# acerbilab/pyvbmc

Measured on AMD Instinct MI355X. Metric: ELBO+entropy evals/sec at D=10, K=50, N=400, Ns=1e6 (1e6-sample-equivalent evals/s), higher is better.
Workload: dtype f64; 1 GPU; BASELINE config 3 per GPU: D=10 K=50 N=400 S=1, Ns=1000000 MC samples per GPU (job Ns=1000000), value+grad _neg_elcbo with soft bounds, eps=philox; parallelism=single GPU

## Files before the change

### pyvbmc_amd/build.py

```python
import os
import subprocess
import sys
from pathlib import Path

HERE = Path(__file__).resolve().parent
CSRC = HERE / "csrc"
LIB = HERE / "libvbmc_hip.so"
SOURCES = [
    "ctx.hip",
    "entropy.hip",
    "entropy_small.hip",
    "prep.hip",
    "api_entropy.hip",
    "mixture.hip",
    "gp.hip",
    "api_gp.hip",
    "gp_post.hip",
    "api_gp_post.hip",
    "gp_lml.hip",
    "api_gp_lml.hip",
    "lockstep.hip",
    "gp_hyp.hip",
    "api_gp_hyp.hip",
    "gp_opt.hip",
    "api_gp_opt.hip",
    "gp_fit.hip",
    "api_gp_fit.hip",
    "api_elbo.hip",
    "api_batch.hip",
    "adam.hip",
    "adam_fused.hip",
    "api_acq.hip",
    "api_acq_is.hip",
    "acq_is_prep.hip",
    "acq_is_mcmc.hip",
    "search.hip",
    "api_search.hip",
    "sieve.hip",
    "api_sieve.hip",
    "elcbo_full.hip",
    "api_elcbo_full.hip",
    "cmaes.hip",
    "api_cmaes.hip",
    "sample.hip",
    "transform.hip",
    "kde.hip",
    "mode.hip",
    "warp.hip",
    "api_warp.hip",
    "comm.hip",
    "host_randn.hip",
    "device_randn.hip",
]
PROBE_SRC = CSRC / "devprobe.hip"
PROBE_LIB = HERE / "libvbmc_devprobe.so"
HIPCC = os.environ.get("HIPCC", "/opt/rocm/bin/hipcc")
FLAGS = [
    "--offload-arch=gfx950",
    "-O3",
    "-std=c++17",
    "-fPIC",
    "-ffp-contract=off",
    "-Wall",
    "-Wno-unused-function",
    "-Werror=pass-failed",
]


WS_DPS = [2, 4, 6, 8, 10, 12, 16, 20, 24, 32]
MFMA_DPS = [12, 16, 20, 24, 32]
WS_EXTRA = os.environ.get("VBMC_WS_EXTRA_FLAGS", "").split()
ALL_EXTRA = os.environ.get("VBMC_EXTRA_FLAGS", "").split()


def _sources():
    return [CSRC / s for s in SOURCES if (CSRC / s).exists()]


SOURCE_FLAGS = {}


def _jobs(bdir):
    jobs = [(src, bdir / (src.stem + ".o"), list(ALL_EXTRA) + SOURCE_FLAGS.get(src.name, [])) for src in _sources()]
    for dp in WS_DPS:
        jobs.append((CSRC / "entropy_ws.hip", bdir / f"entropy_ws_dp{dp}.o", [f"-DVBMC_DP={dp}"] + WS_EXTRA))
    for dp in MFMA_DPS:
        jobs.append((CSRC / "entropy_mfma.hip", bdir / f"entropy_mfma_dp{dp}.o", [f"-DVBMC_MFMA_DP={dp}"] + ALL_EXTRA))
    return jobs


def _headers():
    return list(CSRC.glob("*.h")) + [HERE.parent / "include" / "vbmc_hip.h"]


def _stale(lib, deps):
    return not lib.exists() or any(p.stat().st_mtime > lib.stat().st_mtime for p in deps)


def _lib_stale():
    return _stale(LIB, _sources() + [CSRC / "entropy_ws.hip", CSRC / "entropy_mfma.hip"] + _headers())


def _probe_stale():
    return _stale(PROBE_LIB, [PROBE_SRC] + _headers())


def needs_build():
    return _lib_stale() or _probe_stale()


def build_probe(verbose=True):
    cmd = [HIPCC, *FLAGS, *ALL_EXTRA, "-shared", str(PROBE_SRC), "-o", str(PROBE_LIB), "-Wl,-rpath,/opt/rocm/lib"]
    if verbose:
        print(" ".join(cmd), flush=True)
    subprocess.check_call(cmd)
    return PROBE_LIB


def build(force=False, verbose=True):
    if force or _probe_stale():
        build_probe(verbose)
    if not force and not _lib_stale():
        return LIB
    objs = []
    procs = []
    bdir = CSRC / "_obj"
    bdir.mkdir(exist_ok=True)
    import concurrent.futures as cf

    def run(job):
        src, obj, extra = job
        cmd = [HIPCC, *FLAGS, *extra, "-c", str(src), "-o", str(obj)]
        if verbose:
            print(" ".join(cmd), flush=True)
        p = subprocess.run(cmd, stdout=subprocess.PIPE, stderr=subprocess.STDOUT)
        return obj, p

    jobs = _jobs(bdir)
    with cf.ThreadPoolExecutor(max_workers=max(2, (os.cpu_count() or 4))) as ex:
        results = list(ex.map(run, jobs))
    for (src, obj, _), (_, p) in zip(jobs, results):
        objs.append(obj)
        procs.append((obj, p))
    failed = False
    for src, p in procs:
        out = p.stdout
        if p.returncode != 0:
            failed = True
            sys.stderr.write(f"--- {src.name} failed ---\n{out.decode()}\n")
        elif verbose and out.strip():
            sys.stderr.write(out.decode())
    if failed:
        raise RuntimeError("hipcc failed")
    cmd = [HIPCC, "--offload-arch=gfx950", "-shared", "-fPIC", *map(str, objs), "-o", str(LIB),
           "-ldl", "-Wl,-rpath,/opt/rocm/lib"]
    if verbose:
        print(" ".join(cmd), flush=True)
    subprocess.check_call(cmd)
    return LIB


if __name__ == "__main__":
    build(force="--force" in sys.argv)
    print(LIB)
    print(PROBE_LIB)
```

### pyvbmc_amd/variational_optimization.py

```python
import ctypes as C
import math
import os

import numpy as np

from . import _lib
from ._duck import ctx_of, optimize_mask, upload_vp
from .entropy import DEFAULT_RNG, _even_ns, entlb_vbmc, entmc_vbmc, philox_seed, upload_reference_eps
from .gp import upload_gp


def _soft_bound_loss(x, slb, sub, tol_con=1e-3, compute_grad=False):
    x = np.asarray(x, dtype=np.float64)
    ell = (sub - slb) * tol_con
    below = x < slb
    above = x > sub
    y = 0.0
    dy = np.zeros(x.shape)
    if np.any(below):
        y += 0.5 * np.sum(((slb[below] - x[below]) / ell[below]) ** 2)
        dy[below] = (x[below] - slb[below]) / ell[below] ** 2
    if np.any(above):
        y += 0.5 * np.sum(((x[above] - sub[above]) / ell[above]) ** 2)
        dy[above] = (x[above] - sub[above]) / ell[above] ** 2
    return (y, dy) if compute_grad else y


def _vp_bound_loss(vp, theta, theta_bnd, tol_con=1e-3, compute_grad=True):
    D, K = vp.D, vp.K
    pos = 0
    if vp.optimize_mu:
        mu = theta[: D * K]
        pos = D * K
    else:
        mu = vp.mu.ravel(order="F")
    if vp.optimize_sigma:
        ln_sigma = theta[pos : pos + K]
        pos += K
    else:
        ln_sigma = np.log(vp.sigma.ravel())
    ln_lambd = theta[pos : pos + D] if vp.optimize_lambd else np.log(vp.lambd.ravel())
    ln_scale = np.reshape(ln_lambd, (-1, 1)) + np.reshape(ln_sigma, (1, -1))
    parts = []
    if vp.optimize_mu:
        parts.append(np.ravel(mu))
    if vp.optimize_sigma or vp.optimize_lambd:
        parts.append(ln_scale.ravel(order="F"))
    if vp.optimize_weights:
        parts.append(np.ravel(theta[-K:]))
    ext = np.concatenate(parts)
    lb, ub = theta_bnd["lb"].ravel(), theta_bnd["ub"].ravel()
    if not compute_grad:
        return _soft_bound_loss(ext, lb, ub, tol_con)
    L, dL = _soft_bound_loss(ext, lb, ub, tol_con, compute_grad=True)
    out = []
    pos = 0
    if vp.optimize_mu:
        out.append(dL[: D * K])
        pos = D * K
    if vp.optimize_sigma or vp.optimize_lambd:
        block = np.reshape(dL[pos : pos + D * K], (D, K))
        if vp.optimize_sigma:
            out.append(block.sum(axis=0))
        if vp.optimize_lambd:
            out.append(block.sum(axis=1))
    if vp.optimize_weights:
        out.append(dL[-K:])
    return L, np.concatenate(out)


def _gp_log_joint(vp, gp, grad_flags, avg_flag=True, jacobian_flag=True, compute_var=False,
                  separate_K=False, *, ctx=None):
    if np.isscalar(grad_flags):
        grad_flags = (bool(grad_flags),) * 4
    bits = _lib.flags_to_bits(grad_flags)
    ctx = ctx_of(vp, ctx)
    upload_vp(vp, ctx)
    upload_gp(gp, ctx)
    D, K, S = vp.D, vp.K, len(gp.posteriors)
    jac = bool(jacobian_flag)
    n_dG = (D * K * bool(bits & 1) + jac * (K * bool(bits & 2) + D * bool(bits & 4) + K * bool(bits & 8)))
    averaged = S > 1 and avg_flag
    G = np.empty(S)
    dG = np.empty((n_dG, S)) if bits else None
    varG = np.empty(S) if compute_var else None
    var_ss = C.c_double(0.0)
    I_sk = np.empty((S, K)) if separate_K else None
    J_sjk = np.empty((S, K, K)) if (separate_K and compute_var) else None
    ctx.check(
        ctx._lib.vbmc_gp_log_joint(
            ctx._h, bits, int(bool(avg_flag)), int(jac), int(compute_var), _lib.ptr(G),
            _lib.ptr(dG), _lib.ptr(varG), C.byref(var_ss), _lib.ptr(I_sk), _lib.ptr(J_sjk),
        )
    )
    if averaged:
        G_out = G[0]
        dG_out = dG.ravel()[:n_dG].copy() if bits else None
        varG_out = varG[0] if compute_var else None
    else:
        G_out = G[0] if S == 1 else G
        dG_out = (dG[:, 0].copy() if S == 1 else dG) if bits else None
        varG_out = varG if compute_var else None
    vss = var_ss.value if (averaged and compute_var) else 0
    if separate_K:
        return G_out, dG_out, varG_out, None, vss, I_sk, J_sjk
    return G_out, dG_out, varG_out, None, vss


def _neg_elcbo(theta, gp, vp, beta=0.0, Ns=0, compute_grad=True, compute_var=None, theta_bnd=None,
               _entropy_alpha=0.0, separate_K=False, *, rng=None, seed=None, eps_half=None, ctx=None,
               rows=None):
    fs = _fast_last[0]
    if (fs is not None and fs.vp is vp and fs.gp is gp and fs.bnd is theta_bnd and Ns == fs.Ns and beta == 0.0
            and compute_grad is fs.cg and not compute_var and not separate_K and ctx is fs.ctx_arg and rng == fs.rng
            and eps_half is None and rows is None and type(theta) is np.ndarray and theta.size == fs.n_theta):
        rc = fs.call(theta, seed)
        if rc is not None:
            return rc
    _fast_last[0] = None
    if not math.isfinite(beta):
        beta = 0
    if compute_var is None:
        compute_var = beta != 0
    if compute_grad and beta != 0 and compute_var != 2:
        raise NotImplementedError(
            "Computation of the gradient of ELBO with full variance not supported"
        )
    if separate_K and compute_grad:
        raise ValueError(
            "Computing the gradient of variational parameters and "
            "requesting per-component results at the same time."
        )
    ctx_arg = ctx
    ctx = ctx_of(vp, ctx)
    K, D = vp.K, vp.D

    if separate_K or compute_var or beta != 0:
        if rows is not None:
            raise ValueError("rows= is only supported by the fused evaluation")
        return _neg_elcbo_composed(theta, gp, vp, beta, Ns, compute_grad, compute_var, theta_bnd,
                                   separate_K, rng, seed, eps_half, ctx)

    mask = optimize_mask(vp)
    if mask != 15 or getattr(ctx, "D", None) != D or getattr(ctx, "K", None) != K:
        upload_vp(vp, ctx)
    upload_gp(gp, ctx, lazy=True)
    n_theta = theta.size if type(theta) is np.ndarray else np.size(theta)
    fc = _fused_call(ctx, D, K, n_theta, theta_bnd)
    fc.th[:] = theta
    opts = fc.opts
    ns = _even_ns(Ns) if Ns > 0 else 0
    mode = 0
    if ns > 0:
        mode = DEFAULT_RNG if rng is None else rng
        if rows is not None and (eps_half is not None or mode != "philox"):
            raise ValueError("rows= needs rng='philox' (uploaded draws follow the context's own share)")
        if eps_half is not None or mode == "numpy":
            upload_reference_eps(ctx, K, D, ns, eps_half)
            mode, seed = _lib.EPS_RESIDENT, 0
        elif mode == "philox":
            if seed is None:
                seed = philox_seed(ctx)
            mode = _lib.EPS_PHILOX
        else:
            raise ValueError(f"unknown rng {mode!r}")
    shape = (ns, 1 if compute_grad else 0, mask, mode, rows)
    if shape != fc.shape:
        opts.ns_per_comp, opts.compute_grad, opts.optimize_mask = ns, shape[1], mask
        opts.row_begin, opts.row_count = (0, -1) if rows is None else (int(rows[0]), int(rows[1]))
        opts.eps_mode = mode
        fc.shape = shape
    if ns > 0:
        opts.seed = seed
    fc.side = (vp, theta, mask, K)
    try:
        rc = fc.fn(*fc.args)
        if rc != 0:
            if rc == _lib.W_GP_CHANGED:
                upload_gp(gp, ctx)
                rc = fc.fn(*fc.args)
            if rc != 0:
                ctx.check(rc)
        if fc.side is not None:
            fc.apply_side_effects()
    finally:
        fc.side = None
    if rows is None and eps_half is None and (ns == 0 or mode == _lib.EPS_PHILOX) and type(compute_grad) is bool:
        _fast_last[0] = _FastElbo(ctx_arg, ctx, fc, vp, gp, theta_bnd, Ns, compute_grad, rng, mask, D, K, n_theta, mode)
    return fc.F.value, (fc.dF.copy() if compute_grad else None), fc.G.value, fc.H.value, 0


def _neg_elcbo_batch(thetas, gp, vp, theta_bnd=None, *, ctx=None, return_parts=False):
    ctx = ctx_of(vp, ctx)
    thetas = np.ascontiguousarray(np.atleast_2d(thetas), dtype=np.float64)
    B, n_theta = thetas.shape
    upload_vp(vp, ctx)
    upload_gp(gp, ctx)
    opts = _lib.ElboOpts()
    opts.ns_per_comp, opts.compute_grad, opts.optimize_mask = 0, 0, optimize_mask(vp)
    keep = []
    if theta_bnd is not None:
        lb, ub = _lib.f64(theta_bnd["lb"].ravel()), _lib.f64(theta_bnd["ub"].ravel())
        keep += [lb, ub]
        opts.bnd_lb, opts.bnd_ub, opts.n_bnd = _lib.ptr(lb), _lib.ptr(ub), lb.size
        opts.tol_con = float(theta_bnd["tol_con"])
        opts.weight_threshold = float(theta_bnd.get("weight_threshold", 0.0))
        opts.weight_penalty = float(theta_bnd.get("weight_penalty", 0.0))
    F, G, H = np.empty(B), np.empty(B), np.empty(B)
    ctx.check(
        ctx._lib.vbmc_neg_elcbo_batch(
            ctx._h, _lib.ptr(thetas), B, n_theta, C.byref(opts), _lib.ptr(F), _lib.ptr(G), _lib.ptr(H)
        )
    )
    return (F, G, H) if return_parts else F


_RELEASE_CB = os.environ.get("VBMC_RELEASE_CB", "1") != "0"
_FAST_PATH = os.environ.get("VBMC_FAST_PATH", "1") != "0"
_fast_last = [None]


def clear_fast_path():
    _fast_last[0] = None


class _FastElbo:

    __slots__ = ("ctx_arg", "ctx", "fc", "vp", "gp", "bnd", "Ns", "cg", "rng", "mask", "D", "K", "n_theta", "philox",
                 "lb", "ub", "tol", "wthr", "wpen", "fused_last")

    def __init__(self, ctx_arg, ctx, fc, vp, gp, bnd, Ns, cg, rng, mask, D, K, n_theta, mode):
        self.ctx_arg, self.ctx, self.fc, self.vp, self.gp, self.bnd = ctx_arg, ctx, fc, vp, gp, bnd
        self.Ns, self.cg, self.rng, self.mask, self.D, self.K, self.n_theta = Ns, cg, rng, mask, D, K, n_theta
        self.philox = Ns > 0 and mode == _lib.EPS_PHILOX
        self.fused_last = ctx.__dict__.get("_fused_last")
        if bnd is not None:
            self.lb, self.ub = bnd["lb"], bnd["ub"]
            self.tol, self.wthr, self.wpen = bnd["tol_con"], bnd.get("weight_threshold", 0.0), bnd.get("weight_penalty", 0.0)
            if not fc.direct:
                self.vp = None

    def call(self, theta, seed):
        if not _FAST_PATH:
            return None
        vp, ctx, fc, bnd = self.vp, self.ctx, self.fc, self.bnd
        if (((1 if vp.optimize_mu else 0) | (2 if vp.optimize_sigma else 0) | (4 if vp.optimize_lambd else 0)
             | (8 if vp.optimize_weights else 0)) != self.mask or vp.D != self.D or vp.K != self.K
                or ctx.__dict__.get("_fused_last") is not self.fused_last or getattr(ctx, "D", None) != self.D
                or getattr(ctx, "K", None) != self.K or ctx_of(vp, self.ctx_arg) is not ctx):
            return None
        if self.mask != 15:
            return None
        if bnd is not None and (bnd["lb"] is not self.lb or bnd["ub"] is not self.ub or bnd["tol_con"] != self.tol
                                or bnd.get("weight_threshold", 0.0) != self.wthr or bnd.get("weight_penalty", 0.0) != self.wpen):
            return None
        gp = self.gp
        ps, X = gp.posteriors, gp.X
        quick = [id(ps), id(X), X.shape[0]]
        for p in ps:
            quick += (id(p), id(p.alpha), id(p.hyp))
        if quick != ctx.__dict__.get("_gp_quick"):
            return None
        fc.th[:] = theta
        if self.philox:
            fc.opts.seed = philox_seed(ctx) if seed is None else seed
        fc.side = (vp, theta, self.mask, self.K)
        try:
            rc = fc.fn(*fc.args)
            if rc != 0:
                if rc == _lib.W_GP_CHANGED:
                    upload_gp(gp, ctx)
                    rc = fc.fn(*fc.args)
                if rc != 0:
                    ctx.check(rc)
            if fc.side is not None:
                fc.apply_side_effects()
        finally:
            fc.side = None
        return fc.F.value, (fc.dF.copy() if self.cg else None), fc.G.value, fc.H.value, 0


class _FusedCall:

    def __init__(self, ctx, D, K, n_theta):
        self.th = np.empty(n_theta)
        self.dF = np.empty(n_theta)
        self.mu = np.empty((K, D))
        self.sg, self.lm, self.w, self.eta = np.empty(K), np.empty(D), np.empty(K), np.empty(K)
        self.mu_T, self.sg_row, self.lm_col = self.mu.T, self.sg.reshape(1, -1), self.lm.reshape(-1, 1)
        self.w_row, self.eta_row = self.w.reshape(1, -1), self.eta.reshape(1, -1)
        self.F, self.G, self.H = C.c_double(), C.c_double(), C.c_double()
        o = self.opts = _lib.ElboOpts()
        o.row_begin, o.row_count, o.seed = 0, -1, 0
        self.shape = None
        self.lb_src = self.ub_src = self.lb = self.ub = None
        self.fn = ctx._lib.vbmc_neg_elcbo_call
        self.side = None
        self._cb = C.CFUNCTYPE(None, C.c_void_p)(self._released)
        dp = C.POINTER(C.c_double)
        self.block = _lib.ElboCall(
            _lib.ptr(self.th), n_theta, C.pointer(o), C.cast(C.pointer(self.F), dp), _lib.ptr(self.dF),
            C.cast(C.pointer(self.G), dp), C.cast(C.pointer(self.H), dp), _lib.ptr(self.mu), _lib.ptr(self.sg),
            _lib.ptr(self.lm), _lib.ptr(self.w), _lib.ptr(self.eta),
        )
        self.args = (ctx._h, C.byref(self.block))
        if os.environ.get("VBMC_ELBO_CALL_BLOCK", "1") == "0":
            self.fn = ctx._lib.vbmc_neg_elcbo
            self.args = (
                ctx._h, _lib.ptr(self.th), n_theta, C.byref(o), C.byref(self.F), _lib.ptr(self.dF),
                C.byref(self.G), C.byref(self.H), _lib.ptr(self.mu), _lib.ptr(self.sg), _lib.ptr(self.lm),
                _lib.ptr(self.w), _lib.ptr(self.eta),
            )

    def apply_side_effects(self):
        vp, theta, mask, K = self.side
        vp.mu, vp.sigma, vp.lambd, vp.w = self.mu_T.copy(), self.sg_row.copy(), self.lm_col.copy(), self.w_row.copy()
        if mask & 8:
            vp.eta = self.eta_row.copy()
            if type(theta) is np.ndarray and theta.dtype == self.th.dtype:
                theta[-K:] = self.th[-K:]
        if hasattr(vp, "_mode"):
            vp._mode = None
        self.side = None

    def _released(self, _user):
        if self.side is not None:
            try:
                self.apply_side_effects()
            except Exception:
                pass

    def bind_bounds(self, theta_bnd):
        o = self.opts
        if theta_bnd is None:
            if self.lb is not None:
                o.bnd_lb, o.bnd_ub, o.n_bnd = None, None, 0
                self.lb_src = self.ub_src = self.lb = self.ub = None
            return
        lb, ub = theta_bnd["lb"], theta_bnd["ub"]
        if lb is not self.lb_src or ub is not self.ub_src:
            self.lb, self.ub = _lib.f64(np.ravel(lb)), _lib.f64(np.ravel(ub))
            self.direct = np.shares_memory(self.lb, lb) and np.shares_memory(self.ub, ub)
            self.lb_src, self.ub_src = (lb, ub) if self.direct else (None, None)
            o.bnd_lb, o.bnd_ub, o.n_bnd = _lib.ptr(self.lb), _lib.ptr(self.ub), self.lb.size
        o.tol_con = float(theta_bnd["tol_con"])
        o.weight_threshold = float(theta_bnd.get("weight_threshold", 0.0))
        o.weight_penalty = float(theta_bnd.get("weight_penalty", 0.0))


def _fused_call(ctx, D, K, n_theta, theta_bnd):
    last = ctx.__dict__.get("_fused_last")
    if last is not None and last[0] == D and last[1] == K and last[2] == n_theta:
        fc = last[3]
        fc.bind_bounds(theta_bnd)
        return fc
    cache = ctx.__dict__.setdefault("_fused_cache", {})
    key = (D, K, n_theta)
    fc = cache.get(key)
    if fc is None:
        if len(cache) > 16:
            cache.clear()
        fc = cache[key] = _FusedCall(ctx, D, K, n_theta)
    ctx.__dict__["_fused_last"] = (D, K, n_theta, fc)
    ctx.check(ctx._lib.vbmc_set_release_callback(ctx._h, C.cast(fc._cb, C.c_void_p) if _RELEASE_CB else None, None))
    fc.bind_bounds(theta_bnd)
    return fc


def _neg_elcbo_composed(theta, gp, vp, beta, Ns, compute_grad, compute_var, theta_bnd, separate_K,
                        rng, seed, eps_half, ctx):
    K = vp.K
    vp.set_parameters(theta)
    if vp.optimize_weights:
        tail = theta[-K:]
        tail -= np.amax(tail)
        vp.eta = np.reshape(tail, (1, -1))
    if compute_grad:
        grad_flags = (vp.optimize_mu, vp.optimize_sigma, vp.optimize_lambd, vp.optimize_weights)
    else:
        grad_flags = (False,) * 4
    I_sk = J_sjk = None
    dG = dvarG = None
    if separate_K:
        if compute_var:
            G, _, varG, _, varG_ss, I_sk, J_sjk = _gp_log_joint(vp, gp, grad_flags, 1, 1, compute_var, True, ctx=ctx)
        else:
            G, dG, _, _, _, I_sk, _ = _gp_log_joint(vp, gp, grad_flags, 1, 1, 0, True, ctx=ctx)
            varG = varG_ss = 0
    elif compute_var:
        G, dG, varG, dvarG, varG_ss = _gp_log_joint(vp, gp, grad_flags, 1, 1, compute_var, ctx=ctx)
    else:
        G, dG, _, _, _ = _gp_log_joint(vp, gp, grad_flags, 1, 1, 0, ctx=ctx)
        varG = varG_ss = 0
    if Ns > 0:
        H, dH = entmc_vbmc(vp, Ns, grad_flags, 1, rng=rng, seed=seed, eps_half=eps_half, ctx=ctx)
    else:
        H, dH = entlb_vbmc(vp, grad_flags, 1, ctx=ctx)
    F = -G - H
    if compute_grad:
        dF = -dG - dH
    else:
        dF = None
        dH = None
    varH = 0
    varF = varG + varH if compute_var else 0
    if beta != 0:
        F = F + beta * np.sqrt(varF)
        if compute_grad:
            dF = dF + 0.5 * beta * dvarG / np.sqrt(varF)
    if theta_bnd is not None:
        if compute_grad:
            L, dL = _vp_bound_loss(vp, theta, theta_bnd, tol_con=theta_bnd["tol_con"])
            dF = dF + dL
        else:
            L = _vp_bound_loss(vp, theta, theta_bnd, tol_con=theta_bnd["tol_con"], compute_grad=False)
        F = F + L
        if vp.optimize_weights:
            thresh = theta_bnd["weight_threshold"]
            small = vp.w < thresh
            F = F + np.sum(vp.w * small + thresh * (~small)) * theta_bnd["weight_penalty"]
            if compute_grad:
                ee = np.exp(vp.eta.ravel())
                es = ee.sum()
                wg = theta_bnd["weight_penalty"] * small.ravel()
                dL = np.zeros(dF.shape)
                dL[-K:] = -ee * (ee @ wg) / es**2 + ee * wg / es
                dF = dF + dL
    if separate_K:
        return F, dF, G, H, varF, dH, varG_ss, varG, varH, I_sk, J_sjk
    return F, dF, G, H, varF
```

Baseline: 12270 evals/s.

## Move the fast-path ELBO repeat call into a native CPython extension

Adds a C++ CPython extension that reimplements _FastElbo.call: it runs the cache-validity checks, copies theta into the argument block, and calls the library function pointer directly with the GIL released. This is meant to cut Python and ctypes dispatch overhead on each repeated value+grad evaluation. The Python path stays as a fallback when the extension cannot be built or a re-check fails. In exchange it adds a host C++ build step and considerable reference-counting code that could hide correctness bugs.

Result: faster. 12520 evals/s, median of 6 (+2.0%).

```diff
diff --git a/pyvbmc_amd/build.py b/pyvbmc_amd/build.py
--- a/pyvbmc_amd/build.py
+++ b/pyvbmc_amd/build.py
@@ -1,6 +1,7 @@
 import os
 import subprocess
 import sys
+import sysconfig
 from pathlib import Path
 
 HERE = Path(__file__).resolve().parent
@@ -55,6 +56,9 @@
 PROBE_SRC = CSRC / "devprobe.hip"
 PROBE_LIB = HERE / "libvbmc_devprobe.so"
 HIPCC = os.environ.get("HIPCC", "/opt/rocm/bin/hipcc")
+STEP_DEPS = [CSRC / "pyext_step.cpp", CSRC / "step_lane.h"]
+STEP_LIB = HERE / ("_step_native" + (sysconfig.get_config_var("EXT_SUFFIX") or ".so"))
+HOST_CXX = os.environ.get("CXX", "c++")
 FLAGS = [
     "--offload-arch=gfx950",
     "-O3",
@@ -90,7 +94,7 @@
 
 
 def _headers():
-    return list(CSRC.glob("*.h")) + [HERE.parent / "include" / "vbmc_hip.h"]
+    return [h for h in CSRC.glob("*.h") if h not in STEP_DEPS] + [HERE.parent / "include" / "vbmc_hip.h"]
 
 
 def _stale(lib, deps):
@@ -105,8 +109,38 @@
     return _stale(PROBE_LIB, [PROBE_SRC] + _headers())
 
 
+def _step_stale():
+    return _step_buildable() and _stale(STEP_LIB, STEP_DEPS)
+
+
 def needs_build():
-    return _lib_stale() or _probe_stale()
+    return _lib_stale() or _probe_stale() or _step_stale()
+
+
+def _step_includes():
+    import numpy
+
+    return [sysconfig.get_paths()["include"], numpy.get_include()]
+
+
+def _step_buildable():
+    import shutil
+
+    py, npy = (Path(p) for p in _step_includes())
+    return bool(shutil.which(HOST_CXX)) and (py / "Python.h").exists() and (npy / "numpy" / "arrayobject.h").exists()
+
+
+def build_step(verbose=True):
+    if not _step_buildable():
+        print(f"{STEP_LIB.name}: no host C++ compiler or no Python / NumPy headers; the Python repeat path stays",
+              file=sys.stderr, flush=True)
+        return None
+    cmd = [HOST_CXX, "-O2", "-std=c++17", "-fPIC", "-shared", "-fvisibility=hidden", "-Wall",
+           *(f"-I{p}" for p in _step_includes()), str(STEP_DEPS[0]), "-o", str(STEP_LIB)]
+    if verbose:
+        print(" ".join(cmd), flush=True)
+    subprocess.check_call(cmd)
+    return STEP_LIB
 
 
 def build_probe(verbose=True):
@@ -120,6 +154,8 @@
 def build(force=False, verbose=True):
     if force or _probe_stale():
         build_probe(verbose)
+    if force or _step_stale():
+        build_step(verbose)
     if not force and not _lib_stale():
         return LIB
     objs = []
@@ -164,3 +200,4 @@
     build(force="--force" in sys.argv)
     print(LIB)
     print(PROBE_LIB)
+    print(STEP_LIB)
diff --git a/pyvbmc_amd/csrc/pyext_step.cpp b/pyvbmc_amd/csrc/pyext_step.cpp
--- /dev/null
+++ b/pyvbmc_amd/csrc/pyext_step.cpp
@@ -0,0 +1,514 @@
+#define PY_SSIZE_T_CLEAN
+#include <Python.h>
+#include <structmember.h>
+
+#define NPY_NO_DEPRECATED_API NPY_1_7_API_VERSION
+#include <numpy/arrayobject.h>
+
+#include "step_lane.h"
+
+namespace {
+
+struct FastElbo {
+  PyObject_HEAD
+  PyObject *ctx_arg, *ctx, *fc, *vp, *gp, *bnd, *Ns, *cg, *rng, *mask, *D, *K, *n_theta, *philox, *lb, *ub, *tol, *wthr,
+      *wpen, *fused_last;
+  PyObject* keep;
+  StepLane lane;
+};
+
+#define FE_OBJECTS(X)                                                                                                  \
+  X(ctx_arg) X(ctx) X(fc) X(vp) X(gp) X(bnd) X(Ns) X(cg) X(rng) X(mask) X(D) X(K) X(n_theta) X(philox) X(lb) X(ub)    \
+  X(tol) X(wthr) X(wpen) X(fused_last)
+
+PyObject *g_globals, *g_lib_globals, *g_ctx_of, *g_philox_seed, *s_default_ctx;
+PyObject *s_FAST_PATH, *s_optimize_mu, *s_optimize_sigma, *s_optimize_lambd, *s_optimize_weights, *s_D, *s_K, *s_dict,
+    *s_fused_last, *s_ctx, *s_lb, *s_ub, *s_tol_con, *s_weight_threshold, *s_weight_penalty, *s_get, *s_posteriors, *s_X,
+    *s_shape, *s_gp_quick, *s_alpha, *s_hyp, *s_side, *s_call_py, *s_finish_py, *g_zero_f, *g_zero_i;
+
+int ne(PyObject* a, PyObject* b) {
+  if (PyFloat_CheckExact(a) && PyFloat_CheckExact(b)) return PyFloat_AS_DOUBLE(a) != PyFloat_AS_DOUBLE(b);
+  PyObject* r = PyObject_RichCompare(a, b, Py_NE);
+  if (!r) return -1;
+  const int t = PyObject_IsTrue(r);
+  Py_DECREF(r);
+  return t;
+}
+
+int ne_long(long v, PyObject* obj) {
+  if (PyLong_CheckExact(obj)) {
+    int ovf = 0;
+    const long o = PyLong_AsLongAndOverflow(obj, &ovf);
+    return ovf ? 1 : o != v;
+  }
+  PyObject* pv = PyLong_FromLong(v);
+  if (!pv) return -1;
+  const int t = ne(pv, obj);
+  Py_DECREF(pv);
+  return t;
+}
+
+PyObject* getattr_or_none(PyObject* o, PyObject* name) {
+  PyObject* r = PyObject_GetAttr(o, name);
+  if (!r && PyErr_ExceptionMatches(PyExc_AttributeError)) {
+    PyErr_Clear();
+    r = Py_None;
+    Py_INCREF(r);
+  }
+  return r;
+}
+
+PyObject* map_get(PyObject* m, PyObject* key, PyObject* dflt) {
+  if (PyDict_CheckExact(m)) {
+    PyObject* r = PyDict_GetItemWithError(m, key);
+    if (!r) {
+      if (PyErr_Occurred()) return nullptr;
+      r = dflt;
+    }
+    Py_INCREF(r);
+    return r;
+  }
+  return PyObject_CallMethodObjArgs(m, s_get, key, dflt, nullptr);
+}
+
+PyObject* dict_attr_get(PyObject* o, PyObject* key) {
+  PyObject* d = PyObject_GetAttr(o, s_dict);
+  if (!d) return nullptr;
+  PyObject* r = map_get(d, key, Py_None);
+  Py_DECREF(d);
+  return r;
+}
+
+int attr_true(PyObject* o, PyObject* name) {
+  PyObject* v = PyObject_GetAttr(o, name);
+  if (!v) return -1;
+  const int t = PyObject_IsTrue(v);
+  Py_DECREF(v);
+  return t;
+}
+
+int attr_ne(PyObject* o, PyObject* name, PyObject* want) {
+  PyObject* v = PyObject_GetAttr(o, name);
+  if (!v) return -1;
+  const int t = ne(v, want);
+  Py_DECREF(v);
+  return t;
+}
+
+struct QuickItem {
+  void* id;
+  PyObject* value;
+};
+
+int quick_item_equal(const QuickItem& it, PyObject* stored) {
+  if (it.value) return PyObject_RichCompareBool(it.value, stored, Py_EQ);
+  if (PyLong_CheckExact(stored)) {
+    void* p = PyLong_AsVoidPtr(stored);
+    if (!p && PyErr_Occurred()) {
+      PyErr_Clear();
+      return 0;
+    }
+    return p == it.id;
+  }
+  PyObject* v = PyLong_FromVoidPtr(it.id);
+  if (!v) return -1;
+  const int e = PyObject_RichCompareBool(v, stored, Py_EQ);
+  Py_DECREF(v);
+  return e;
+}
+
+int gp_quick_differs(PyObject* gp, PyObject* ctx) {
+  PyObject *ps = nullptr, *X = nullptr, *shape = nullptr, *n0 = nullptr, *stored = nullptr, *it = nullptr;
+  QuickItem small[3 + 3 * 8];
+  QuickItem* items = small;
+  Py_ssize_t n = 0, cap = sizeof(small) / sizeof(small[0]);
+  int out = -1;
+  do {
+    if (!(ps = PyObject_GetAttr(gp, s_posteriors))) break;
+    if (!(X = PyObject_GetAttr(gp, s_X))) break;
+    if (!(shape = PyObject_GetAttr(X, s_shape))) break;
+    if (!(n0 = PySequence_GetItem(shape, 0))) break;
+    items[n++] = {ps, nullptr};
+    items[n++] = {X, nullptr};
+    items[n++] = {nullptr, n0};
+    if (!(it = PyObject_GetIter(ps))) break;
+    bool bad = false;
+    while (PyObject* p = PyIter_Next(it)) {
+      if (n + 3 > cap) {
+        QuickItem* grown = static_cast<QuickItem*>(PyMem_Malloc(sizeof(QuickItem) * 2 * cap));
+        if (!grown) {
+          PyErr_NoMemory();
+          Py_DECREF(p);
+          bad = true;
+          break;
+        }
+        for (Py_ssize_t i = 0; i < n; ++i) grown[i] = items[i];
+        if (items != small) PyMem_Free(items);
+        items = grown;
+        cap *= 2;
+      }
+      PyObject* a = PyObject_GetAttr(p, s_alpha);
+      PyObject* h = a ? PyObject_GetAttr(p, s_hyp) : nullptr;
+      items[n++] = {p, nullptr};
+      items[n++] = {a, nullptr};
+      items[n++] = {h, nullptr};
+      Py_XDECREF(h);
+      Py_XDECREF(a);
+      Py_DECREF(p);
+      if (!a || !h) {
+        bad = true;
+        break;
+      }
+    }
+    if (bad || PyErr_Occurred()) break;
+    if (!(stored = dict_attr_get(ctx, s_gp_quick))) break;
+    if (!PyList_Check(stored) || PyList_GET_SIZE(stored) != n) {
+      out = 1;
+      break;
+    }
+    out = 0;
+    for (Py_ssize_t i = 0; i < n && out == 0; ++i) {
+      if (i >= PyList_GET_SIZE(stored)) {
+        out = 1;
+        break;
+      }
+      PyObject* si = PyList_GET_ITEM(stored, i);
+      Py_INCREF(si);
+      const int e = quick_item_equal(items[i], si);
+      Py_DECREF(si);
+      out = e < 0 ? -1 : !e;
+    }
+  } while (false);
+  if (items != small) PyMem_Free(items);
+  Py_XDECREF(it);
+  Py_XDECREF(stored);
+  Py_XDECREF(n0);
+  Py_XDECREF(shape);
+  Py_XDECREF(X);
+  Py_XDECREF(ps);
+  return out;
+}
+
+PyObject* ctx_of(PyObject* vp, PyObject* ctx_arg) {
+  if (ctx_arg != Py_None) {
+    Py_INCREF(ctx_arg);
+    return ctx_arg;
+  }
+  PyObject* own = getattr_or_none(vp, s_ctx);
+  if (!own || own != Py_None) return own;
+  Py_DECREF(own);
+  PyObject* dflt = PyDict_GetItemWithError(g_lib_globals, s_default_ctx);
+  if (dflt && dflt != Py_None) {
+    Py_INCREF(dflt);
+    return dflt;
+  }
+  if (!dflt && PyErr_Occurred()) return nullptr;
+  return PyObject_CallFunctionObjArgs(g_ctx_of, vp, ctx_arg, nullptr);
+}
+
+bool plain_vector(PyObject* theta, int64_t n) {
+  if (!PyArray_CheckExact(theta)) return false;
+  PyArrayObject* a = reinterpret_cast<PyArrayObject*>(theta);
+  return PyArray_TYPE(a) == NPY_DOUBLE && PyArray_ISNOTSWAPPED(a) && PyArray_NDIM(a) == 1 && PyArray_DIM(a, 0) == n &&
+         PyArray_IS_C_CONTIGUOUS(a) && PyArray_ISALIGNED(a);
+}
+
+PyObject* fe_call(PyObject* self_, PyObject* const* args, Py_ssize_t nargs) {
+  FastElbo* s = reinterpret_cast<FastElbo*>(self_);
+  if (nargs != 2) {
+    PyErr_SetString(PyExc_TypeError, "call(theta, seed)");
+    return nullptr;
+  }
+  PyObject *theta = args[0], *seed = args[1];
+  if (!s->lane.fn || !plain_vector(theta, s->lane.n_theta) || !(seed == Py_None || PyLong_CheckExact(seed)))
+    return PyObject_CallMethodObjArgs(self_, s_call_py, theta, seed, nullptr);
+#define NEED(f)                                                \
+  if (!s->f) {                                                 \
+    PyErr_SetString(PyExc_AttributeError, #f);                 \
+    return nullptr;                                            \
+  }
+  NEED(vp) NEED(ctx) NEED(fc) NEED(bnd) NEED(mask) NEED(D) NEED(K) NEED(fused_last) NEED(ctx_arg) NEED(gp) NEED(philox)
+  NEED(cg)
+#undef NEED
+  PyObject* fp = PyDict_GetItemWithError(g_globals, s_FAST_PATH);
+  if (!fp) {
+    if (!PyErr_Occurred()) PyErr_SetString(PyExc_NameError, "name '_FAST_PATH' is not defined");
+    return nullptr;
+  }
+  int t = PyObject_IsTrue(fp);
+  if (t < 0) return nullptr;
+  if (!t) Py_RETURN_NONE;
+  PyObject *vp = s->vp, *ctx = s->ctx, *fc = s->fc, *bnd = s->bnd;
+#define TRY(expr)            \
+  if ((t = (expr)) < 0) return nullptr;
+#define NONE_IF(expr)        \
+  TRY(expr)                  \
+  if (t) Py_RETURN_NONE;
+  long mask = 0;
+  TRY(attr_true(vp, s_optimize_mu)) mask |= t ? 1 : 0;
+  TRY(attr_true(vp, s_optimize_sigma)) mask |= t ? 2 : 0;
+  TRY(attr_true(vp, s_optimize_lambd)) mask |= t ? 4 : 0;
+  TRY(attr_true(vp, s_optimize_weights)) mask |= t ? 8 : 0;
+  NONE_IF(ne_long(mask, s->mask))
+  NONE_IF(attr_ne(vp, s_D, s->D))
+  NONE_IF(attr_ne(vp, s_K, s->K))
+  {
+    PyObject* fl = dict_attr_get(ctx, s_fused_last);
+    if (!fl) return nullptr;
+    const bool same = fl == s->fused_last;
+    Py_DECREF(fl);
+    if (!same) Py_RETURN_NONE;
+    PyObject* v = getattr_or_none(ctx, s_D);
+    if (!v) return nullptr;
+    t = ne(v, s->D);
+    Py_DECREF(v);
+    NONE_IF(t)
+    if (!(v = getattr_or_none(ctx, s_K))) return nullptr;
+    t = ne(v, s->K);
+    Py_DECREF(v);
+    NONE_IF(t)
+    if (!(v = ctx_of(vp, s->ctx_arg))) return nullptr;
+    const bool is_ctx = v == ctx;
+    Py_DECREF(v);
+    if (!is_ctx) Py_RETURN_NONE;
+  }
+  NONE_IF(ne_long(15, s->mask))
+  if (bnd != Py_None) {
+    PyObject* v = PyObject_GetItem(bnd, s_lb);
+    if (!v) return nullptr;
+    bool other = v != s->lb;
+    Py_DECREF(v);
+    if (other) Py_RETURN_NONE;
+    if (!(v = PyObject_GetItem(bnd, s_ub))) return nullptr;
+    other = v != s->ub;
+    Py_DECREF(v);
+    if (other) Py_RETURN_NONE;
+    if (!s->tol || !s->wthr || !s->wpen) {
+      PyErr_SetString(PyExc_AttributeError, "tol");
+      return nullptr;
+    }
+    if (!(v = PyObject_GetItem(bnd, s_tol_con))) return nullptr;
+    t = ne(v, s->tol);
+    Py_DECREF(v);
+    NONE_IF(t)
+    if (!(v = map_get(bnd, s_weight_threshold, g_zero_f))) return nullptr;
+    t = ne(v, s->wthr);
+    Py_DECREF(v);
+    NONE_IF(t)
+    if (!(v = map_get(bnd, s_weight_penalty, g_zero_f))) return nullptr;
+    t = ne(v, s->wpen);
+    Py_DECREF(v);
+    NONE_IF(t)
+  }
+  NONE_IF(gp_quick_differs(s->gp, ctx))
+  step_lane_pack(s->lane, static_cast<const double*>(PyArray_DATA(reinterpret_cast<PyArrayObject*>(theta))));
+  TRY(PyObject_IsTrue(s->cg))
+  const int cg = t;
+  TRY(PyObject_IsTrue(s->philox))
+  if (t) {
+    if (seed == Py_None) {
+      PyObject* sd = PyObject_CallFunctionObjArgs(g_philox_seed, ctx, nullptr);
+      if (!sd) return nullptr;
+      const unsigned long long v = PyLong_AsUnsignedLongLongMask(sd);
+      Py_DECREF(sd);
+      if (v == static_cast<unsigned long long>(-1) && PyErr_Occurred()) return nullptr;
+      *s->lane.seed = v;
+    } else {
+      const unsigned long long v = PyLong_AsUnsignedLongLongMask(seed);
+      if (v == static_cast<unsigned long long>(-1) && PyErr_Occurred()) return nullptr;
+      *s->lane.seed = v;
+    }
+  }
+  {
+    PyObject* side = PyTuple_Pack(4, vp, theta, s->mask, s->K);
+    if (!side) return nullptr;
+    const int rc = PyObject_SetAttr(fc, s_side, side);
+    Py_DECREF(side);
+    if (rc < 0) return nullptr;
+  }
+  const StepLane lane = s->lane;
+  Py_INCREF(self_);
+  Py_INCREF(fc);
+  int rc;
+  Py_BEGIN_ALLOW_THREADS
+  rc = step_lane_invoke(lane);
+  Py_END_ALLOW_THREADS
+  PyObject* out = nullptr;
+  do {
+    if (PyErr_Occurred()) {
+      PyObject *et, *ev, *tb;
+      PyErr_Fetch(&et, &ev, &tb);
+      if (PyObject_SetAttr(fc, s_side, Py_None) < 0) PyErr_Clear();
+      PyErr_Restore(et, ev, tb);
+      break;
+    }
+    PyObject* side = PyObject_GetAttr(fc, s_side);
+    if (!side) break;
+    const bool applied = side == Py_None;
+    Py_DECREF(side);
+    if (rc != 0 || !applied) {
+      PyObject* prc = PyLong_FromLong(rc);
+      if (!prc) break;
+      out = PyObject_CallMethodObjArgs(self_, s_finish_py, prc, nullptr);
+      Py_DECREF(prc);
+      break;
+    }
+    PyObject *F = PyFloat_FromDouble(*lane.F), *G = PyFloat_FromDouble(*lane.G), *H = PyFloat_FromDouble(*lane.H);
+    PyObject* dF = nullptr;
+    if (cg) {
+      npy_intp n = static_cast<npy_intp>(lane.n_theta);
+      dF = PyArray_SimpleNew(1, &n, NPY_DOUBLE);
+      if (dF) step_lane_grad(lane, static_cast<double*>(PyArray_DATA(reinterpret_cast<PyArrayObject*>(dF))));
+    } else {
+      dF = Py_None;
+      Py_INCREF(dF);
+    }
+    if (F && G && H && dF) out = PyTuple_Pack(5, F, dF, G, H, g_zero_i);
+    Py_XDECREF(F);
+    Py_XDECREF(G);
+    Py_XDECREF(H);
+    Py_XDECREF(dF);
+  } while (false);
+  Py_DECREF(fc);
+  Py_DECREF(self_);
+  return out;
+#undef TRY
+#undef NONE_IF
+}
+
+PyObject* fe_bind(PyObject* self_, PyObject* args) {
+  FastElbo* s = reinterpret_cast<FastElbo*>(self_);
+  unsigned long long fn, handle, block, F, G, H, seed;
+  PyObject *th, *dF, *keep;
+  if (!PyArg_ParseTuple(args, "KKKOOKKKKO", &fn, &handle, &block, &th, &dF, &F, &G, &H, &seed, &keep)) return nullptr;
+  if (!PyArray_CheckExact(th) || !PyArray_CheckExact(dF)) {
+    PyErr_SetString(PyExc_TypeError, "th and dF must be ndarrays");
+    return nullptr;
+  }
+  PyArrayObject *a = reinterpret_cast<PyArrayObject*>(th), *b = reinterpret_cast<PyArrayObject*>(dF);
+  if (PyArray_NDIM(a) != 1 || !plain_vector(dF, PyArray_DIM(a, 0)) || !plain_vector(th, PyArray_DIM(a, 0)) ||
+      !PyArray_ISWRITEABLE(a) || !fn || !block || !F || !G || !H || !seed) {
+    PyErr_SetString(PyExc_ValueError, "the argument block's theta and dF must be float64 vectors of one length");
+    return nullptr;
+  }
+  PyObject* held = PyTuple_Pack(3, th, dF, keep);
+  if (!held) return nullptr;
+  Py_XSETREF(s->keep, held);
+  StepLane& l = s->lane;
+  l.fn = reinterpret_cast<int (*)(void*, const void*)>(static_cast<uintptr_t>(fn));
+  l.handle = reinterpret_cast<void*>(static_cast<uintptr_t>(handle));
+  l.block = reinterpret_cast<const void*>(static_cast<uintptr_t>(block));
+  l.th = static_cast<double*>(PyArray_DATA(a));
+  l.dF = static_cast<const double*>(PyArray_DATA(b));
+  l.F = reinterpret_cast<const double*>(static_cast<uintptr_t>(F));
+  l.G = reinterpret_cast<const double*>(static_cast<uintptr_t>(G));
+  l.H = reinterpret_cast<const double*>(static_cast<uintptr_t>(H));
+  l.seed = reinterpret_cast<uint64_t*>(static_cast<uintptr_t>(seed));
+  l.n_theta = PyArray_DIM(a, 0);
+  Py_RETURN_NONE;
+}
+
+int fe_traverse(PyObject* self_, visitproc visit, void* arg) {
+  FastElbo* s = reinterpret_cast<FastElbo*>(self_);
+#define X(f) Py_VISIT(s->f);
+  FE_OBJECTS(X)
+#undef X
+  Py_VISIT(s->keep);
+  return 0;
+}
+
+int fe_clear(PyObject* self_) {
+  FastElbo* s = reinterpret_cast<FastElbo*>(self_);
+  s->lane = StepLane();
+#define X(f) Py_CLEAR(s->f);
+  FE_OBJECTS(X)
+#undef X
+  Py_CLEAR(s->keep);
+  return 0;
+}
+
+void fe_dealloc(PyObject* self_) {
+  PyObject_GC_UnTrack(self_);
+  fe_clear(self_);
+  Py_TYPE(self_)->tp_free(self_);
+}
+
+PyMemberDef fe_members[] = {
+#define X(f) {#f, T_OBJECT_EX, offsetof(FastElbo, f), 0, nullptr},
+    FE_OBJECTS(X)
+#undef X
+    {nullptr, 0, 0, 0, nullptr}};
+
+PyMethodDef fe_methods[] = {
+    {"call", reinterpret_cast<PyCFunction>(reinterpret_cast<void (*)()>(fe_call)), METH_FASTCALL,
+     "call(theta, seed): the repeat of the last fused _neg_elcbo call, or None when a re-check fails"},
+    {"_bind_lane", fe_bind, METH_VARARGS, "addresses of the argument block the record repeats"},
+    {nullptr, nullptr, 0, nullptr}};
+
+PyTypeObject FastElboType = {PyVarObject_HEAD_INIT(nullptr, 0)};
+
+PyObject* mod_setup(PyObject*, PyObject* args) {
+  PyObject *globals, *lib_globals, *ctx_of_fn, *philox_fn;
+  if (!PyArg_ParseTuple(args, "O!O!OO", &PyDict_Type, &globals, &PyDict_Type, &lib_globals, &ctx_of_fn, &philox_fn))
+    return nullptr;
+  Py_INCREF(globals);
+  Py_INCREF(lib_globals);
+  Py_XSETREF(g_lib_globals, lib_globals);
+  Py_INCREF(ctx_of_fn);
+  Py_INCREF(philox_fn);
+  Py_XSETREF(g_globals, globals);
+  Py_XSETREF(g_ctx_of, ctx_of_fn);
+  Py_XSETREF(g_philox_seed, philox_fn);
+  Py_RETURN_NONE;
+}
+
+PyMethodDef mod_methods[] = {
+    {"setup", mod_setup, METH_VARARGS,
+     "setup(module globals holding _FAST_PATH, _lib's globals holding _default_ctx, ctx_of, philox_seed)"},
+    {nullptr, nullptr, 0, nullptr}};
+
+PyModuleDef mod_def = {PyModuleDef_HEAD_INIT, "_step_native", "native repeat lane of _neg_elcbo", -1, mod_methods,
+                       nullptr, nullptr, nullptr, nullptr};
+
+}
+
+PyMODINIT_FUNC PyInit__step_native(void) {
+  import_array();
+  struct {
+    PyObject** slot;
+    const char* text;
+  } names[] = {{&s_FAST_PATH, "_FAST_PATH"}, {&s_optimize_mu, "optimize_mu"}, {&s_optimize_sigma, "optimize_sigma"},
+               {&s_optimize_lambd, "optimize_lambd"}, {&s_optimize_weights, "optimize_weights"}, {&s_D, "D"}, {&s_K, "K"},
+               {&s_dict, "__dict__"}, {&s_fused_last, "_fused_last"}, {&s_ctx, "_ctx"}, {&s_lb, "lb"}, {&s_ub, "ub"},
+               {&s_tol_con, "tol_con"}, {&s_weight_threshold, "weight_threshold"}, {&s_weight_penalty, "weight_penalty"},
+               {&s_get, "get"}, {&s_posteriors, "posteriors"}, {&s_X, "X"}, {&s_shape, "shape"}, {&s_gp_quick, "_gp_quick"},
+               {&s_alpha, "alpha"}, {&s_hyp, "hyp"}, {&s_side, "side"}, {&s_call_py, "_call_py"},
+               {&s_finish_py, "_finish_py"}, {&s_default_ctx, "_default_ctx"}};
+  for (auto& n : names)
+    if (!(*n.slot = PyUnicode_InternFromString(n.text))) return nullptr;
+  if (!(g_zero_f = PyFloat_FromDouble(0.0)) || !(g_zero_i = PyLong_FromLong(0))) return nullptr;
+  FastElboType.tp_name = "pyvbmc_amd._step_native.FastElboBase";
+  FastElboType.tp_basicsize = sizeof(FastElbo);
+  FastElboType.tp_flags = Py_TPFLAGS_DEFAULT | Py_TPFLAGS_BASETYPE | Py_TPFLAGS_HAVE_GC;
+  FastElboType.tp_doc = "what a repeat of the last fused _neg_elcbo call needs, and the repeat itself";
+  FastElboType.tp_new = PyType_GenericNew;
+  FastElboType.tp_dealloc = fe_dealloc;
+  FastElboType.tp_traverse = fe_traverse;
+  FastElboType.tp_clear = fe_clear;
+  FastElboType.tp_members = fe_members;
+  FastElboType.tp_methods = fe_methods;
+  if (PyType_Ready(&FastElboType) < 0) return nullptr;
+  PyObject* m = PyModule_Create(&mod_def);
+  if (!m) return nullptr;
+  if (PyModule_AddIntConstant(m, "ABI", 1) < 0) {
+    Py_DECREF(m);
+    return nullptr;
+  }
+  Py_INCREF(&FastElboType);
+  if (PyModule_AddObject(m, "FastElboBase", reinterpret_cast<PyObject*>(&FastElboType)) < 0) {
+    Py_DECREF(&FastElboType);
+    Py_DECREF(m);
+    return nullptr;
+  }
+  return m;
+}
diff --git a/pyvbmc_amd/csrc/step_lane.h b/pyvbmc_amd/csrc/step_lane.h
--- /dev/null
+++ b/pyvbmc_amd/csrc/step_lane.h
@@ -0,0 +1,24 @@
+#pragma once
+#include <cstdint>
+#include <cstring>
+
+struct StepLane {
+  int (*fn)(void*, const void*) = nullptr;
+  void* handle = nullptr;
+  const void* block = nullptr;
+  double* th = nullptr;
+  const double* dF = nullptr;
+  const double *F = nullptr, *G = nullptr, *H = nullptr;
+  uint64_t* seed = nullptr;
+  int64_t n_theta = 0;
+};
+
+static inline void step_lane_pack(const StepLane& l, const double* src) {
+  std::memmove(l.th, src, sizeof(double) * static_cast<size_t>(l.n_theta));
+}
+
+static inline int step_lane_invoke(const StepLane& l) { return l.fn(l.handle, l.block); }
+
+static inline void step_lane_grad(const StepLane& l, double* dst) {
+  std::memcpy(dst, l.dF, sizeof(double) * static_cast<size_t>(l.n_theta));
+}
diff --git a/pyvbmc_amd/variational_optimization.py b/pyvbmc_amd/variational_optimization.py
--- a/pyvbmc_amd/variational_optimization.py
+++ b/pyvbmc_amd/variational_optimization.py
@@ -224,10 +224,26 @@
     _fast_last[0] = None
 
 
-class _FastElbo:
-
-    __slots__ = ("ctx_arg", "ctx", "fc", "vp", "gp", "bnd", "Ns", "cg", "rng", "mask", "D", "K", "n_theta", "philox",
-                 "lb", "ub", "tol", "wthr", "wpen", "fused_last")
+_FAST_FIELDS = ("ctx_arg", "ctx", "fc", "vp", "gp", "bnd", "Ns", "cg", "rng", "mask", "D", "K", "n_theta", "philox",
+                "lb", "ub", "tol", "wthr", "wpen", "fused_last")
+
+_step_native = None
+if os.environ.get("VBMC_NATIVE_LANE", "1") != "0":
+    try:
+        from . import _step_native
+    except ImportError:
+        _step_native = None
+    if getattr(_step_native, "ABI", None) != 1:
+        _step_native = None
+
+
+class _FastElboFields:
+    __slots__ = _FAST_FIELDS
+
+
+class _FastElbo(_FastElboFields if _step_native is None else _step_native.FastElboBase):
+
+    __slots__ = ()
 
     def __init__(self, ctx_arg, ctx, fc, vp, gp, bnd, Ns, cg, rng, mask, D, K, n_theta, mode):
         self.ctx_arg, self.ctx, self.fc, self.vp, self.gp, self.bnd = ctx_arg, ctx, fc, vp, gp, bnd
@@ -239,8 +255,13 @@
             self.tol, self.wthr, self.wpen = bnd["tol_con"], bnd.get("weight_threshold", 0.0), bnd.get("weight_penalty", 0.0)
             if not fc.direct:
                 self.vp = None
-
-    def call(self, theta, seed):
+        if _step_native is not None and fc.block_call:
+            o = fc.opts
+            self._bind_lane(C.cast(fc.fn, C.c_void_p).value, ctx._h.value, C.addressof(fc.block), fc.th, fc.dF,
+                            C.addressof(fc.F), C.addressof(fc.G), C.addressof(fc.H),
+                            C.addressof(o) + _lib.ElboOpts.seed.offset, (fc.block, o, fc.F, fc.G, fc.H, fc.fn))
+
+    def _call_py(self, theta, seed):
         if not _FAST_PATH:
             return None
         vp, ctx, fc, bnd = self.vp, self.ctx, self.fc, self.bnd
@@ -267,9 +288,17 @@
         fc.side = (vp, theta, self.mask, self.K)
         try:
             rc = fc.fn(*fc.args)
+        except BaseException:
+            fc.side = None
+            raise
+        return self._finish_py(rc)
+
+    def _finish_py(self, rc):
+        ctx, fc = self.ctx, self.fc
+        try:
             if rc != 0:
                 if rc == _lib.W_GP_CHANGED:
-                    upload_gp(gp, ctx)
+                    upload_gp(self.gp, ctx)
                     rc = fc.fn(*fc.args)
                 if rc != 0:
                     ctx.check(rc)
@@ -278,6 +307,12 @@
         finally:
             fc.side = None
         return fc.F.value, (fc.dF.copy() if self.cg else None), fc.G.value, fc.H.value, 0
+
+
+if _step_native is None:
+    _FastElbo.call = _FastElbo._call_py
+else:
+    _step_native.setup(globals(), vars(_lib), ctx_of, philox_seed)
 
 
 class _FusedCall:
@@ -304,8 +339,10 @@
             _lib.ptr(self.lm), _lib.ptr(self.w), _lib.ptr(self.eta),
         )
         self.args = (ctx._h, C.byref(self.block))
+        self.block_call = True
         if os.environ.get("VBMC_ELBO_CALL_BLOCK", "1") == "0":
             self.fn = ctx._lib.vbmc_neg_elcbo
+            self.block_call = False
             self.args = (
                 ctx._h, _lib.ptr(self.th), n_theta, C.byref(o), C.byref(self.F), _lib.ptr(self.dF),
                 C.byref(self.G), C.byref(self.H), _lib.ptr(self.mu), _lib.ptr(self.sg), _lib.ptr(self.lm),
```
